# david-mathews-1994/deltarice

Hardware: AMD Instinct MI355X
Metric: encode+decode GB/s (int16 in) (higher is better)
Workload: dtype int16; 1 GPU; 1000000x7000 int16 Gaussian(sigma=10), m=8, 500 chunks of 2000x7000 per GPU, encode then decode, HBM resident; waveforms_per_gpu=1000000, wave_len=7000, rice_m=8, chunks_per_gpu=500, decode_impl=8

## Files before the change

### deltarice_amd/csrc/drx_encode.h

```cpp
#ifndef DRX_ENCODE_H
#define DRX_ENCODE_H
#include <hip/hip_runtime.h>
#include <stdint.h>

#include "drx_device.h"

namespace drx {

constexpr int kTile = 512;

typedef uint16_t u16x2 __attribute__((ext_vector_type(2)));
typedef int16_t i16x2 __attribute__((ext_vector_type(2)));
__device__ __forceinline__ u16x2 as_u16x2(uint32_t x) { return __builtin_bit_cast(u16x2, x); }
__device__ __forceinline__ i16x2 as_i16x2(uint32_t x) { return __builtin_bit_cast(i16x2, x); }
__device__ __forceinline__ uint32_t as_u32(u16x2 x) { return __builtin_bit_cast(uint32_t, x); }
__device__ __forceinline__ u16x2 splat(uint32_t v) { return (u16x2){(uint16_t)v, (uint16_t)v}; }

struct PackedCodes { uint32_t nb[4], c16[4], e[4]; };

template <bool GEN>
__device__ __forceinline__ void packed_codes(const uint32_t x[4], uint32_t xprev, uint32_t xprev2, const u16x2 (&tp)[4],
                                             uint32_t k, PackedCodes &c) {
    const u16x2 kv = splat(k), kp1 = splat(k + 1u), c16k = splat(16u - k);
    const u16x2 mlo = splat((1u << k) - 1u), mdelta = splat(0xffffu - ((1u << k) - 1u));
    u16x2 z[4], qc[4], e[4];
#pragma unroll
    for (int j = 0; j < 4; ++j) {
        const uint32_t xm1 = j ? x[j - 1] : xprev;
        const uint32_t before = __builtin_amdgcn_alignbit(x[j], xm1, 16);
        i16x2 d;
        if (GEN) {
            const uint32_t xm2 = j >= 2 ? x[j - 2] : (j == 1 ? xprev : xprev2);
            const uint32_t before3 = __builtin_amdgcn_alignbit(xm1, xm2, 16);
            d = __builtin_bit_cast(i16x2, (u16x2)(as_u16x2(x[j]) * tp[0] + as_u16x2(before) * tp[1] +
                                                  as_u16x2(xm1) * tp[2] + as_u16x2(before3) * tp[3]));
        } else {
            d = as_i16x2(x[j]) - as_i16x2(before);
        }
        z[j] = __builtin_bit_cast(u16x2, (i16x2)(d << (int16_t)1)) ^
               __builtin_bit_cast(u16x2, (i16x2)(d >> (int16_t)15));
    }
#pragma unroll
    for (int j = 0; j < 4; ++j) qc[j] = __builtin_elementwise_min((u16x2)(z[j] >> kv), splat(8u));
#pragma unroll
    for (int j = 0; j < 4; ++j) e[j] = qc[j] >> (uint16_t)3;
#pragma unroll
    for (int j = 0; j < 4; ++j) c.nb[j] = as_u32(e[j] * c16k + (qc[j] + kp1));
    const uint32_t mword = as_u32(splat(1u << k));
#pragma unroll
    for (int j = 0; j < 4; ++j) {
        const uint32_t mask = as_u32(e[j] * mdelta + mlo);
        c.c16[j] = (mask & as_u32(z[j])) | (~mask & mword);
        c.e[j] = as_u32(e[j]);
    }
}

constexpr uint32_t kEncCapWords = 2048;

__device__ __forceinline__ int load8_dwords(const int16_t *__restrict__ x, uint32_t len, uint32_t t0, int lane,
                                            bool vec_ok, uint32_t w[4]) {
    const uint32_t i0 = t0 + 8u * (uint32_t)lane;
    const int nv = (i0 >= len) ? 0 : (int)((len - i0) < 8u ? (len - i0) : 8u);
    if (vec_ok && nv == 8) {
        const uint4 q = *reinterpret_cast<const uint4 *>(x + i0);
        w[0] = q.x; w[1] = q.y; w[2] = q.z; w[3] = q.w;
    } else {
#pragma unroll
        for (int j = 0; j < 4; ++j) {
            const uint32_t a = (2 * j < nv) ? (uint32_t)(uint16_t)x[i0 + 2 * j] : 0u;
            const uint32_t b = (2 * j + 1 < nv) ? (uint32_t)(uint16_t)x[i0 + 2 * j + 1] : 0u;
            w[j] = a | (b << 16);
        }
    }
    return nv;
}

__device__ __forceinline__ void mask_tail(PackedCodes &c, int nv) {
#pragma unroll
    for (int j = 0; j < 4; ++j) {
        const uint32_t m = (2 * j + 1 < nv) ? 0xffffffffu : ((2 * j < nv) ? 0x0000ffffu : 0u);
        c.nb[j] &= m;
    }
}

__device__ __forceinline__ uint32_t lane_tile_bits(const PackedCodes &c) {
    const u16x2 s = as_u16x2(c.nb[0]) + as_u16x2(c.nb[1]) + as_u16x2(c.nb[2]) + as_u16x2(c.nb[3]);
    const uint32_t v = as_u32(s);
    return (v & 0xffffu) + (v >> 16);
}

template <bool FULL>
__device__ __forceinline__ void emit_tile(const PackedCodes &c, uint32_t pb) {
    typedef uint32_t __attribute__((address_space(3))) lds_u32;
#pragma unroll
    for (int j = 0; j < 8; ++j) {
        const uint32_t n = (j & 1) ? (c.nb[j >> 1] >> 16) : (c.nb[j >> 1] & 0xffffu);
        uint32_t code32 = __builtin_amdgcn_perm(c.e[j >> 1], c.c16[j >> 1], (j & 1) ? 0x07060302u : 0x05040100u);
        if (!FULL) code32 = n ? code32 : 0u;
        const uint32_t pe = pb + n;
        const uint64_t v = (uint64_t)code32 << (((pb & 32u) - pe) & 63u);
        lds_u32 *w = (lds_u32 *)(uintptr_t)((pb >> 3) & ~3u);
        __hip_atomic_fetch_or(w, (uint32_t)(v >> 32), __ATOMIC_RELAXED, __HIP_MEMORY_SCOPE_WORKGROUP);
        if ((uint32_t)v) __hip_atomic_fetch_or(w + 1, (uint32_t)v, __ATOMIC_RELAXED, __HIP_MEMORY_SCOPE_WORKGROUP);
        pb = pe;
    }
}

__device__ __forceinline__ void concat_codes(const PackedCodes &c, uint32_t (&w)[4]) {
    uint32_t w0 = 0, w1 = 0, w2 = 0, w3 = 0;
#pragma unroll
    for (int j = 0; j < 8; ++j) {
        const uint32_t nbj = c.nb[j >> 1];
        const uint32_t n = (j & 1) ? (nbj >> 16) : nbj;
        const uint32_t code32 = __builtin_amdgcn_perm(c.e[j >> 1], c.c16[j >> 1], (j & 1) ? 0x07060302u : 0x05040100u);
        const uint32_t s = 0u - n;
        if (j >= 3) w3 = __builtin_amdgcn_alignbit(w3, w2, s);
        if (j >= 2) w2 = __builtin_amdgcn_alignbit(w2, w1, s);
        if (j >= 1) w1 = __builtin_amdgcn_alignbit(w1, w0, s);
        w0 = (w0 << (n & 31u)) | code32;
    }
    w[0] = w0; w[1] = w1; w[2] = w2; w[3] = w3;
}

__device__ __forceinline__ void place_words(const uint32_t (&wd)[4], uint32_t pe) {
    typedef uint32_t __attribute__((address_space(3))) lds_u32;
    const uint32_t x0 = __builtin_amdgcn_alignbit(wd[0], 0u, pe);
    const uint32_t x1 = __builtin_amdgcn_alignbit(wd[1], wd[0], pe);
    const uint32_t x2 = __builtin_amdgcn_alignbit(wd[2], wd[1], pe);
    const uint32_t x3 = __builtin_amdgcn_alignbit(wd[3], wd[2], pe);
    const uint32_t x4 = __builtin_amdgcn_alignbit(0u, wd[3], pe);
    lds_u32 *w = (lds_u32 *)(uintptr_t)(((pe >> 3) & ~3u) - 16u);
    __hip_atomic_fetch_or(w + 4, x0, __ATOMIC_RELAXED, __HIP_MEMORY_SCOPE_WORKGROUP);
    __hip_atomic_fetch_or(w + 3, x1, __ATOMIC_RELAXED, __HIP_MEMORY_SCOPE_WORKGROUP);
    __hip_atomic_fetch_or(w + 2, x2, __ATOMIC_RELAXED, __HIP_MEMORY_SCOPE_WORKGROUP);
    if (x3 | x4) {
        __hip_atomic_fetch_or(w + 1, x3, __ATOMIC_RELAXED, __HIP_MEMORY_SCOPE_WORKGROUP);
        if (x4) __hip_atomic_fetch_or(w, x4, __ATOMIC_RELAXED, __HIP_MEMORY_SCOPE_WORKGROUP);
    }
}

constexpr uint32_t kBufFront = 4;

__device__ __forceinline__ void zero_row(uint32_t *row, uint32_t words, int lane) {
    for (int i = lane; i < (int)(words / 4u); i += 64) reinterpret_cast<uint4 *>(row)[i] = make_uint4(0, 0, 0, 0);
}

struct TileCodes {
    PackedCodes c;
    uint32_t cw[4], lane_bits, incl, tile_bits;
};

template <bool GEN, bool FULLT>
__device__ __forceinline__ TileCodes code_tile(const uint32_t (&w)[4], int nv, uint32_t &carry, uint32_t &carry2, const u16x2 (&tp)[4],
                                               uint32_t k) {
    TileCodes t;
    const uint32_t xprev = wave_shr1_carry(w[3], carry);
    carry = (uint32_t)__builtin_amdgcn_readlane((int)w[3], 63);
    uint32_t xprev2 = 0;
    if (GEN) {
        xprev2 = wave_shr1_carry(w[2], carry2);
        carry2 = (uint32_t)__builtin_amdgcn_readlane((int)w[2], 63);
    }
    packed_codes<GEN>(w, xprev, xprev2, tp, k, t.c);
    if (!FULLT) mask_tail(t.c, nv);
    t.lane_bits = lane_tile_bits(t.c);
    if (FULLT) concat_codes(t.c, t.cw);
    t.incl = wave_incl_scan_dpp(t.lane_bits);
    t.tile_bits = (uint32_t)__builtin_amdgcn_readlane((int)t.incl, 63);
    return t;
}

template <bool FULLT, typename At>
__device__ __forceinline__ void put_tile(const TileCodes &t, At &&at) {
    if (FULLT && !__any(t.lane_bits > 128u))
        place_words(t.cw, at(t.incl));
    else
        emit_tile<FULLT>(t.c, at(t.incl - t.lane_bits));
}

__device__ __forceinline__ void shr128(uint32_t (&w)[4], uint32_t n) {
    const uint32_t ws = n >> 5;
    const uint32_t y0 = ws == 0u ? w[0] : ws == 1u ? w[1] : ws == 2u ? w[2] : ws == 3u ? w[3] : 0u;
    const uint32_t y1 = ws == 0u ? w[1] : ws == 1u ? w[2] : ws == 2u ? w[3] : 0u;
    const uint32_t y2 = ws == 0u ? w[2] : ws == 1u ? w[3] : 0u;
    const uint32_t y3 = ws == 0u ? w[3] : 0u;
    w[0] = __builtin_amdgcn_alignbit(y1, y0, n);
    w[1] = __builtin_amdgcn_alignbit(y2, y1, n);
    w[2] = __builtin_amdgcn_alignbit(y3, y2, n);
    w[3] = y3 >> (n & 31u);
}

template <bool GEN>
__device__ __forceinline__ TileCodes code_tail_tile(const uint32_t (&w)[4], int nv, bool ragged, uint32_t &carry, uint32_t &carry2,
                                                    const u16x2 (&tp)[4], uint32_t k, bool &wide) {
    TileCodes t;
    const uint32_t xprev = wave_shr1_carry(w[3], carry);
    carry = (uint32_t)__builtin_amdgcn_readlane((int)w[3], 63);
    uint32_t xprev2 = 0;
    if (GEN) {
        xprev2 = wave_shr1_carry(w[2], carry2);
        carry2 = (uint32_t)__builtin_amdgcn_readlane((int)w[2], 63);
    }
    packed_codes<GEN>(w, xprev, xprev2, tp, k, t.c);
    const uint32_t all_bits = lane_tile_bits(t.c);
    concat_codes(t.c, t.cw);
    if (ragged) {
        PackedCodes cm = t.c;
        mask_tail(cm, nv);
        t.lane_bits = lane_tile_bits(cm);
        shr128(t.cw, all_bits - t.lane_bits);
    } else {
        t.lane_bits = nv ? all_bits : 0u;
#pragma unroll
        for (int j = 0; j < 4; ++j) t.cw[j] = nv ? t.cw[j] : 0u;
    }
    wide = __any((nv ? all_bits : 0u) > 128u);
    t.incl = wave_incl_scan_dpp(t.lane_bits);
    t.tile_bits = (uint32_t)__builtin_amdgcn_readlane((int)t.incl, 63);
    return t;
}

template <typename At>
__device__ __forceinline__ void put_tail_tile(const TileCodes &t, int nv, bool wide, At &&at) {
    if (!wide) {
        place_words(t.cw, at(t.incl));
    } else {
        PackedCodes c = t.c;
        mask_tail(c, nv);
        emit_tile<false>(c, at(t.incl - t.lane_bits));
    }
}

template <typename B, typename F>
__device__ __forceinline__ void for_full_tiles(const int16_t *__restrict__ x, uint32_t n_full, int lane, B &&between, F &&full) {
    constexpr int kDepth = 3;
    const uint4 *xv = reinterpret_cast<const uint4 *>(x) + lane;
    uint4 q[kDepth];
    uint32_t t = 0;
#pragma unroll
    for (int u = 0; u < kDepth; ++u) {
        q[u] = make_uint4(0, 0, 0, 0);
        if ((uint32_t)u < n_full) q[u] = xv[64 * (size_t)u];
    }
#pragma unroll 1
    for (; t + 2u * kDepth <= n_full; t += kDepth) {
        between();
#pragma unroll
        for (int u = 0; u < kDepth; ++u) {
            const uint32_t w[4] = {q[u].x, q[u].y, q[u].z, q[u].w};
            full(w);
            q[u] = xv[64 * (size_t)(t + u + kDepth)];
        }
    }
#pragma unroll 1
    for (; t < n_full; t += kDepth) {
        between();
#pragma unroll
        for (int u = 0; u < kDepth; ++u) {
            if (t + (uint32_t)u < n_full) {
                const uint32_t w[4] = {q[u].x, q[u].y, q[u].z, q[u].w};
                full(w);
                if (t + (uint32_t)u + kDepth < n_full) q[u] = xv[64 * (size_t)(t + u + kDepth)];
            }
        }
    }
}

template <typename B, typename F, typename T>
__device__ __forceinline__ void for_tiles(const int16_t *__restrict__ x, uint32_t len, uint32_t n_full, bool tail, int lane,
                                          B &&between, F &&full, T &&tailf) {
    constexpr int kDepth = 3;
    const uint32_t last = tail ? n_full : n_full - 1u;
    const uint32_t imax = len - 8u;
    auto load = [&](uint32_t tile) -> uint4 {
        tile = tile < last ? tile : last;
        uint32_t i = tile * (uint32_t)kTile + 8u * (uint32_t)lane;
        i = i < imax ? i : imax;
        return *reinterpret_cast<const uint4 *>(x + i);
    };
    uint4 q[kDepth];
#pragma unroll
    for (int u = 0; u < kDepth; ++u) {
        q[u] = load((uint32_t)u);
        __builtin_amdgcn_sched_barrier(0);
    }
    uint32_t t = 0;
#pragma unroll 1
    for (; t + kDepth <= n_full; t += kDepth) {
        between(true);
#pragma unroll
        for (int u = 0; u < kDepth; ++u) {
            const uint32_t w[4] = {q[u].x, q[u].y, q[u].z, q[u].w};
            full(w);
            q[u] = load(t + (uint32_t)u + kDepth);
        }
    }
    const uint32_t left = n_full - t;
    static_assert(kDepth == 3, "the straight code below");
    if (left) {
        between(false);
        const uint32_t w0[4] = {q[0].x, q[0].y, q[0].z, q[0].w};
        full(w0);
        if (left > 1u) {
            const uint32_t w1[4] = {q[1].x, q[1].y, q[1].z, q[1].w};
            full(w1);
        }
    }
    if (tail) {
        auto sel = [left](uint32_t a, uint32_t b, uint32_t c) -> uint32_t { return left == 0u ? a : (left == 1u ? b : c); };
        const uint32_t w[4] = {sel(q[0].x, q[1].x, q[2].x), sel(q[0].y, q[1].y, q[2].y), sel(q[0].z, q[1].z, q[2].z),
                               sel(q[0].w, q[1].w, q[2].w)};
        tailf(w);
    } else {
        __builtin_amdgcn_s_waitcnt(0x0f70);
    }
}

template <bool GEN, bool WINDOW>
__device__ __forceinline__ uint64_t recode_tiles(const int16_t *__restrict__ x, uint32_t len, uint32_t carry, uint32_t carry2,
                                                 const u16x2 (&tp)[4], uint32_t k, int lane, uint32_t *row, uint32_t row_words,
                                                 uint32_t *__restrict__ outp, uint32_t P0, uint32_t skip, uint32_t limit, uint64_t cap) {
    zero_row(row, row_words, lane);
    wave_sync();
    uint32_t *buf = row + kBufFront;
    const uint32_t buf_bits = lds_addr(buf) * 8u;
    auto mine = [&](uint64_t idx) -> bool { return !WINDOW || (idx >= skip && idx < limit && idx < cap); };
    uint64_t P = P0;
    uint32_t wn[4];
    int nvn = load8_dwords(x, len, 0u, lane, true, wn);
    for (uint32_t t0 = 0; t0 < len; t0 += kTile) {
        const uint32_t w[4] = {wn[0], wn[1], wn[2], wn[3]};
        const int nv = nvn;
        if (t0 + kTile < len) nvn = load8_dwords(x, len, t0 + kTile, lane, true, wn);
        const TileCodes t = code_tile<GEN, false>(w, nv, carry, carry2, tp, k);
        const uint64_t wfirst = P >> 5;
        const uint32_t at0 = buf_bits + (uint32_t)(P & 31u);
        put_tile<false>(t, [&](uint32_t bit) -> uint32_t { return at0 + bit; });
        P += t.tile_bits;
        wave_sync();
        const uint32_t nfull = (uint32_t)((P >> 5) - wfirst);
        for (uint32_t i = lane; i < nfull; i += 64) {
            if (mine(wfirst + i)) outp[wfirst + i] = buf[i];
            buf[i] = 0;
        }
        wave_sync();
        if (nfull && lane == 0) { const uint32_t cwd = buf[nfull]; buf[nfull] = 0; buf[0] = cwd; }
        wave_sync();
    }
    if (lane == 0) {
        if ((P & 31u) && mine(P >> 5)) outp[P >> 5] = buf[0];
        buf[0] = 0;
    }
    wave_sync();
    return P;
}

template <bool GEN>
__device__ __forceinline__ uint64_t recode_waveform(const int16_t *__restrict__ x, uint32_t len, const u16x2 (&tp)[4], uint32_t k, int lane,
                                                    uint32_t *row, uint32_t row_words, uint32_t *__restrict__ outp) {
    return recode_tiles<GEN, false>(x, len, 0u, 0u, tp, k, lane, row, row_words, outp, 0u, 0u, 0u, 0ull);
}

template <bool GEN>
__device__ __forceinline__ void history_before(const int16_t *__restrict__ x, uint32_t &carry, uint32_t &carry2) {
    carry = (uint32_t)(uint16_t)x[-1] << 16;
    if (GEN) {
        carry |= (uint32_t)(uint16_t)x[-2];
        carry2 = (uint32_t)(uint16_t)x[-4] | ((uint32_t)(uint16_t)x[-3] << 16);
    }
}

template <bool GEN>
__device__ __forceinline__ void recode_range(const int16_t *__restrict__ xw, uint32_t wf_len, uint32_t s_begin, uint32_t s_end, uint64_t Bp,
                                             uint32_t bits_mine, const u16x2 (&tp)[4], uint32_t k, int lane, uint32_t *row,
                                             uint32_t row_words, uint32_t *__restrict__ payload, uint64_t cap_words) {
    const uint32_t P0 = (uint32_t)(Bp & 31u);
    const uint64_t wbase = Bp >> 5;
    const uint32_t more = wf_len - s_end < 32u ? wf_len - s_end : 32u;
    uint32_t carry = 0, carry2 = 0;
    if (s_begin) history_before<GEN>(xw + s_begin, carry, carry2);
    recode_tiles<GEN, true>(xw + s_begin, s_end - s_begin + more, carry, carry2, tp, k, lane, row, row_words, payload + wbase, P0,
                            P0 ? 1u : 0u, (P0 + bits_mine + 31u) >> 5, cap_words > wbase ? cap_words - wbase : 0ull);
}

}
#endif
```

### deltarice_amd/csrc/drx_encode_stream.hip

```cpp
#include <hip/hip_runtime.h>
#include <stdint.h>

#include <type_traits>

#include "drx_internal.h"
#include "drx_device.h"
#include "drx_encode.h"

namespace drx {

constexpr int kEsWaves = 4;
constexpr uint32_t kEsFront = kBufFront;
constexpr uint32_t kEsBack = 12;
constexpr uint64_t kEsFlag = 1ull << 63;
constexpr uint32_t kEsCtrlWords = 32;
constexpr uint32_t kEsRing = kEsRingWords;
constexpr int kEsPollSleep = 4;

__device__ __forceinline__ uint64_t es_load(const uint64_t *p) {
    return __hip_atomic_load(p, __ATOMIC_RELAXED, __HIP_MEMORY_SCOPE_AGENT);
}
__device__ __forceinline__ void es_store(uint64_t *p, uint64_t v) {
    __hip_atomic_store(p, v, __ATOMIC_RELAXED, __HIP_MEMORY_SCOPE_AGENT);
}

constexpr uint32_t kScPer = 8;

__device__ __forceinline__ void es_scanner(uint64_t total, const uint64_t *__restrict__ size, uint64_t *__restrict__ place,
                                           DevStatus *st) {
    const int lane = lane_id();
    if (threadIdx.x >= 64) return;
    __builtin_amdgcn_s_setprio(3);
    uint64_t pos = 0, base = 0;
    uint32_t idle = 0;
    auto sample = [&](uint64_t (&v)[kScPer], uint64_t at) {
#pragma unroll
        for (int j = 0; j < (int)kScPer; ++j) {
            const uint64_t e = at + 64u * j + (uint32_t)lane;
            v[j] = e < total ? es_load(size + e) : kEsFlag;
        }
    };
    while (pos < total) {
        uint64_t v[kScPer];
        const uint64_t bs = pos;
        sample(v, pos);
        uint64_t run = 0;
        bool open = true, big = false;
#pragma unroll
        for (int j = 0; j < (int)kScPer; ++j) {
            const uint64_t e = bs + 64u * j + (uint32_t)lane;
            const uint64_t m = __ballot(e < pos || (v[j] >> 63) != 0);
            const uint32_t l = (m == ~0ull) ? 64u : (uint32_t)__builtin_ctzll(~m);
            run += open ? l : 0u;
            open = open && l == 64u;
            big = big || __any((v[j] & ~kEsFlag) >= (1ull << 24));
        }
        uint64_t end = bs + run;
        end = end < total ? end : total;
        if (end <= pos) {
            if (++idle > (1u << 22)) {
                if (lane == 0) atomicOr(&st->err, kErrInternal);
                return;
            }
            __builtin_amdgcn_s_sleep(1);
            continue;
        }
        idle = 0;
        uint64_t running = 0;
#pragma unroll
        for (int j = 0; j < (int)kScPer; ++j) {
            if (bs + 64u * j < end) {
                const uint64_t e = bs + 64u * j + (uint32_t)lane;
                const bool in = e >= pos && e < end;
                const uint64_t val = in ? (v[j] & ~kEsFlag) : 0ull;
                uint64_t inc;
                if (!big) {
                    inc = wave_incl_scan_dpp((uint32_t)val);
                } else {
                    inc = val;
#pragma unroll
                    for (int d = 1; d < 64; d <<= 1) {
                        const uint64_t t = __shfl_up(inc, d);
                        if (lane >= d) inc += t;
                    }
                }
                if (in) es_store(place + e, kEsFlag | (base + running + inc - val));
                running += big ? __shfl(inc, 63) : (uint64_t)(uint32_t)__builtin_amdgcn_readlane((int)(uint32_t)inc, 63);
            }
        }
        base += running;
        pos = end;
    }
}

template <int WV>
struct EsShared {
    uint32_t role, arrive, ticket[4];
    uint64_t mine[2][WV];
    uint32_t place_t[2];
};

template <int WV>
__device__ __forceinline__ uint32_t es_rendezvous(EsShared<WV> &shm, uint32_t cyc, int lane, int wv, uint32_t *__restrict__ ctrl,
                                                  uint64_t *__restrict__ size, uint32_t Tprev, uint64_t &off) {
    typedef uint32_t __attribute__((address_space(3))) lds_u32;
    uint32_t arr = 0;
    if (lane == 0) arr = __hip_atomic_fetch_add((lds_u32 *)&shm.arrive, 1u, __ATOMIC_RELAXED, __HIP_MEMORY_SCOPE_WORKGROUP);
    arr = (uint32_t)__builtin_amdgcn_readfirstlane((int)arr);
    if (arr == (uint32_t)WV * cyc) {
        if (lane == 0) shm.ticket[cyc & 3u] = atomicAdd(ctrl + 32, 1u);
    }
    __syncthreads();
    const uint32_t T = rfl(shm.ticket[cyc & 3u]);
    if (cyc) {
        uint64_t sum = 0, before = 0;
#pragma unroll
        for (int i = 0; i < WV; ++i) {
            const uint64_t m = rfl64(shm.mine[(cyc - 1u) & 1u][i]);
            sum += m;
            before += i < wv ? m : 0ull;
        }
        off = before;
        if (wv == 0 && lane == 0) es_store(size + Tprev, kEsFlag | sum);
    }
    return T;
}

template <uint32_t RING>
__device__ __forceinline__ uint32_t es_gap(bool pend, uint32_t startA, uint32_t start, uint32_t behind) {
    if (!pend) return RING - 8u;
    const uint32_t d = startA >= start ? startA - start : startA + RING - start;
    return d > behind ? d - behind : 0u;
}

template <typename InLds, typename Wait, typename Copy>
__device__ __forceinline__ bool es_release(bool must, uint64_t P, InLds &&place_in_lds, Wait &&wait_place, Copy &&copy_out) {
    decltype(wait_place()) pl;
    const bool seen = place_in_lds(pl);
    if (!(seen || must)) return false;
    if (!seen) __builtin_amdgcn_s_setprio(0);
    else if (P < (uint64_t)(4u * kTile * 7u)) __builtin_amdgcn_s_setprio(2);
    else __builtin_amdgcn_s_setprio(1);
    copy_out(seen ? pl : wait_place());
    return true;
}

template <uint32_t RING, typename Put>
__device__ __forceinline__ void ring_put_with(const TileCodes &t, uint32_t *row, uint32_t s0, int lane, Put &&put) {
    constexpr uint32_t kRingBits = RING * 32u;
    uint32_t *ring = row + kEsFront;
    const uint32_t ring_bits0 = lds_addr(ring) * 8u;
    put([&](uint32_t bit) -> uint32_t {
        const uint32_t b = s0 + bit;
        return ring_bits0 + (b >= kRingBits ? b - kRingBits : b);
    });
    if (s0 < kRingBits && s0 + t.tile_bits >= kRingBits) {
        wave_sync();
        if (lane < (int)kEsFront) {
            const uint32_t v = row[lane];
            if (v) { ring[RING - kEsFront + lane] |= v; row[lane] = 0; }
        } else if (lane < (int)(kEsFront + kEsBack)) {
            const uint32_t i = (uint32_t)lane - kEsFront, v = ring[RING + i];
            if (v) { ring[i] |= v; ring[RING + i] = 0; }
        }
        wave_sync();
    }
}
template <bool FULLT, uint32_t RING>
__device__ __forceinline__ void ring_put(const TileCodes &t, uint32_t *row, uint32_t s0, int lane) {
    ring_put_with<RING>(t, row, s0, lane, [&](auto &&at) { put_tile<FULLT>(t, at); });
}

static unsigned es_grid(const Geom &G, uint64_t tickets) {
    const unsigned full = 256u * (16u / kEsWaves);
    return (G.dbg & DRX_DBG_STREAM_THREE_WGS) ? 3u : (unsigned)(tickets + 1 < full ? tickets + 1 : full);
}

template <bool GEN, int WV, uint32_t RING>
__global__ __launch_bounds__(64 * WV, 4) void k_encode_stream(Geom G, const int16_t *__restrict__ in, uint32_t *__restrict__ out,
                                                              uint64_t out_cap, uint64_t *__restrict__ chunk_word_off,
                                                              uint32_t *__restrict__ wave_words, uint64_t *__restrict__ size,
                                                              uint64_t *__restrict__ place, uint32_t *__restrict__ ctrl,
                                                              DevStatus *st) {
    __shared__ __attribute__((aligned(16))) uint32_t ring_all[WV][kEsFront + RING + kEsBack];
    __shared__ EsShared<WV> shm;
    __shared__ uint64_t s_place_v[2];
    typedef uint32_t __attribute__((address_space(3))) lds_u32;
    typedef uint64_t __attribute__((address_space(3))) lds_u64;
    static_assert((kEsFront + RING + kEsBack) % 4 == 0 && RING % 4 == 0, "16-byte LDS accesses");
    constexpr uint32_t kRowWords = kEsFront + RING + kEsBack;
    const int lane = lane_id(), wv = wave_id();
    uint32_t *row = ring_all[wv];
    uint32_t *ring = row + kEsFront;

    if (threadIdx.x == 0) {
        shm.role = atomicAdd(ctrl, 1u);
        shm.arrive = 0;
        shm.place_t[0] = shm.place_t[1] = 0;
    }
    zero_row(row, kRowWords, lane);
    __syncthreads();
    const uint64_t n_tickets = (G.total_waves + WV - 1) / WV;
    if (rfl(shm.role) == 0) {
        es_scanner(n_tickets, size, place, st);
        return;
    }

    const uint32_t k = G.k;
    const u16x2 tp[4] = {splat(GEN ? G.enc_t[0] : 1u), splat(GEN ? G.enc_t[1] : 0xffffu), splat(GEN ? G.enc_t[2] : 0u),
                         splat(GEN ? G.enc_t[3] : 0u)};

    bool pend = false, fitsA = true;
    uint64_t gA = 0, offA = 0;
    uint32_t TA = 0, startA = 0, nA = 0;
    WaveRef rA = {};

    auto place_header = [&](const WaveRef &r, uint64_t g, uint32_t n, uint64_t ex, uint64_t &pos) -> bool {
        const uint64_t mine = 1ull + n + (r.idx == 0 ? 1ull : 0ull);
        pos = ex + (r.idx == 0 ? 1ull : 0ull);
        if (lane == 0) {
            if (r.idx == 0) chunk_word_off[r.chunk] = ex;
            if (g + 1 == G.total_waves) {
                chunk_word_off[G.n_chunks] = ex + mine;
                st->total_words = ex + mine;
                if (G.host_words) *G.host_words = ex + mine;
                if (ex + mine > out_cap) atomicOr(&st->err, kErrCapacity);
            }
        }
        const bool room = pos + 1u + n <= out_cap;
        if (room && lane == 0) {
            out[pos] = n;
            if (r.idx == 0) out[pos - 1] = r.n_samples;
        }
        return room;
    };
    auto copy_out = [&](uint64_t ex) {
        uint64_t pos;
        const bool room = place_header(rA, gA, nA, ex + offA, pos);
        uint32_t *__restrict__ outp = out + pos + 1;
        typedef uint32_t u32x4s __attribute__((ext_vector_type(4)));
        typedef u32x4s __attribute__((address_space(1), aligned(4))) g_u32x4_a4;
        const uint32_t n4 = nA & ~3u;
        for (uint32_t i = 4u * (uint32_t)lane; i < n4; i += 256u) {
            uint32_t w = startA + i;
            w = w >= RING ? w - RING : w;
            const uint4 v = *reinterpret_cast<const uint4 *>(ring + w);
            if (room) *(g_u32x4_a4 *)(outp + i) = (u32x4s){v.x, v.y, v.z, v.w};
            *reinterpret_cast<uint4 *>(ring + w) = make_uint4(0, 0, 0, 0);
        }
        if ((uint32_t)lane < nA - n4) {
            uint32_t w = startA + n4 + (uint32_t)lane;
            w = w >= RING ? w - RING : w;
            if (room) outp[n4 + (uint32_t)lane] = ring[w];
            ring[w] = 0;
        }
        wave_sync();
        pend = false;
    };
    auto place_in_lds = [&](uint64_t &ex) -> bool {
        const uint32_t t = __hip_atomic_load((lds_u32 *)&shm.place_t[TA & 1u], __ATOMIC_RELAXED, __HIP_MEMORY_SCOPE_WORKGROUP);
        if (rfl(t) != TA + 1u) return false;
        ex = rfl64(__hip_atomic_load((lds_u64 *)&s_place_v[TA & 1u], __ATOMIC_RELAXED, __HIP_MEMORY_SCOPE_WORKGROUP));
        return true;
    };
    auto place_to_lds = [&](uint64_t ex) {
        if (lane == 0) {
            __hip_atomic_store((lds_u64 *)&s_place_v[TA & 1u], ex, __ATOMIC_RELAXED, __HIP_MEMORY_SCOPE_WORKGROUP);
            __hip_atomic_store((lds_u32 *)&shm.place_t[TA & 1u], TA + 1u, __ATOMIC_RELAXED, __HIP_MEMORY_SCOPE_WORKGROUP);
        }
    };
    auto wait_place = [&]() -> uint64_t {
        uint32_t spins = 0;
        for (;;) {
            uint64_t ex;
            bool have = place_in_lds(ex);
            if (!have) {
                uint64_t v = 0;
                if (lane == 0) v = es_load(place + TA);
                const uint32_t hi = (uint32_t)__builtin_amdgcn_readfirstlane((int)(uint32_t)(v >> 32));
                if (hi >> 31) {
                    ex = ((uint64_t)(hi & 0x7fffffffu) << 32) | (uint32_t)__builtin_amdgcn_readfirstlane((int)(uint32_t)v);
                    place_to_lds(ex);
                    have = true;
                }
            }
            if (have) return ex;
            __builtin_amdgcn_s_sleep(kEsPollSleep);
            if (++spins > (1u << 22)) {
                if (lane == 0) atomicOr(&st->err, kErrInternal);
                return out_cap;
            }
        }
    };

    auto stream_out = [&](uint64_t ex) {
        uint64_t pos;
        const bool room = place_header(rA, gA, nA, ex + offA, pos);
        recode_waveform<GEN>(in + rA.sample_off, room ? rA.len : 0u, tp, k, lane, row, kRowWords, out + pos + 1);
        pend = false;
    };

    uint32_t start = 0;
    uint32_t Tprev = 0;
    for (uint32_t cyc = 0;; ++cyc) {
        const uint32_t T = es_rendezvous(shm, cyc, lane, wv, ctrl, size, Tprev, offA);
        if (pend && !fitsA) stream_out(wait_place());
        if ((uint64_t)T * WV >= G.total_waves) break;
        Tprev = T;
        const uint64_t g = (uint64_t)T * WV + (uint32_t)wv;
        if (g >= G.total_waves) {
            if (lane == 0) shm.mine[cyc & 1u][wv] = 0;
            if (pend) copy_out(wait_place());
            continue;
        }

        const WaveRef r = locate_uniform(G, g);
        const int16_t *x = in + r.sample_off;
        const uint32_t wlen = r.len;
        const uint32_t n_full = wlen / kTile, rem = wlen - n_full * (uint32_t)kTile;
        const bool tail = rem != 0u, ragged = (rem & 7u) != 0u;
        const bool tail_lane = 8u * (uint32_t)lane + 8u <= rem;

        auto gap = [&]() -> uint32_t { return es_gap<RING>(pend, startA, start, 8u); };
        if (pend && gap() < 512u) copy_out(wait_place());
        uint32_t limit = gap();

        uint64_t P = 0;
        bool fits = true;
        uint32_t carry = 0;
        uint32_t carry2 = 0;
        auto process_tile = [&](const uint32_t (&w)[4], int nv, auto full_tag) {
            constexpr bool FULLT = decltype(full_tag)::value;
            bool wide = false;
            TileCodes t;
            if constexpr (FULLT) t = code_tile<GEN, true>(w, nv, carry, carry2, tp, k);
            else t = code_tail_tile<GEN>(w, nv, ragged, carry, carry2, tp, k, wide);
            const uint32_t need = ((uint32_t)P + t.tile_bits + 31u) >> 5;
            bool ok = fits && need < limit;
            if (pend && es_release(fits && !ok, P, place_in_lds, wait_place, copy_out)) {
                limit = gap();
                ok = fits && need < limit;
            }
            if (ok) {
                if constexpr (FULLT) ring_put<true, RING>(t, row, start * 32u + (uint32_t)P, lane);
                else ring_put_with<RING>(t, row, start * 32u + (uint32_t)P, lane, [&](auto &&at) { put_tail_tile(t, nv, wide, at); });
            } else {
                fits = false;
            }
            P += t.tile_bits;
        };
        uint64_t pollv = 0;
        bool polling = false;
        auto between = [&](bool again) {
            if (!pend) return;
            if (polling) {
                const uint32_t hi = (uint32_t)__builtin_amdgcn_readfirstlane((int)(uint32_t)(pollv >> 32));
                polling = false;
                if (hi >> 31) {
                    place_to_lds(((uint64_t)(hi & 0x7fffffffu) << 32) | (uint32_t)__builtin_amdgcn_readfirstlane((int)(uint32_t)pollv));
                    return;
                }
            }
            if (!again) return;
            if (lane == 0) pollv = es_load(place + TA);
            polling = true;
        };

        auto full_tile = [&](const uint32_t (&w)[4]) { process_tile(w, 8, std::true_type{}); };
        auto tail_tile = [&](const uint32_t (&wq)[4]) {
            const uint32_t i0 = 8u * (uint32_t)lane;
            const int nv = tail_lane ? 8 : (i0 < rem ? (int)(rem - i0) : 0);
            uint32_t w[4];
#pragma unroll
            for (int j = 0; j < 4; ++j) w[j] = tail_lane ? wq[j] : 0u;
            if (ragged && nv > 0 && nv < 8) {
                const int16_t *xl = x + (size_t)n_full * kTile + i0;
#pragma unroll
                for (int j = 0; j < 4; ++j) {
                    const uint32_t a = (2 * j < nv) ? (uint32_t)(uint16_t)xl[2 * j] : 0u;
                    const uint32_t b = (2 * j + 1 < nv) ? (uint32_t)(uint16_t)xl[2 * j + 1] : 0u;
                    w[j] = a | (b << 16);
                }
            }
            process_tile(w, nv, std::false_type{});
        };
        if (wlen >= 8u) {
            for_tiles(x, wlen, n_full, tail, lane, between, full_tile, tail_tile);
        } else {
            const uint32_t none[4] = {0u, 0u, 0u, 0u};
            tail_tile(none);
        }
        const uint32_t n = (uint32_t)((P + 31u) >> 5);
        wave_sync();
        if (lane == 0) {
            wave_words[g] = n;
            shm.mine[cyc & 1u][wv] = 1ull + n + (r.idx == 0 ? 1ull : 0ull);
        }
        if (pend) copy_out(wait_place());
        pend = true;
        fitsA = fits;
        gA = g;
        rA = r;
        TA = T;
        startA = start;
        nA = n;
        if (fits) {
            start += (n + 3u) & ~3u;
            start = start >= RING ? start - RING : start;
        }
    }
    if (pend) copy_out(wait_place());
}

struct EsPlace2 { uint64_t whdr, bits; };

__device__ __forceinline__ void es_scanner_segs(uint64_t total, uint32_t tpw, uint32_t waves_per_chunk, const uint64_t *__restrict__ size,
                                                uint64_t *__restrict__ place, DevStatus *st) {
    const int lane = lane_id();
    if (threadIdx.x >= 64) return;
    __builtin_amdgcn_s_setprio(3);
    uint64_t pos = 0;
    uint64_t whdr = 1;
    uint64_t bits_in = 0;
    uint32_t idle = 0;
    const double rcp_tpw = 1.0 / (double)tpw;
    while (pos < total) {
        uint64_t v[kScPer];
        const uint64_t bs = pos;
#pragma unroll
        for (int j = 0; j < (int)kScPer; ++j) {
            const uint64_t e = bs + 64u * j + (uint32_t)lane;
            v[j] = e < total ? es_load(size + e) : 0ull;
        }
        uint64_t run = 0;
        bool open = true;
#pragma unroll
        for (int j = 0; j < (int)kScPer; ++j) {
            const uint64_t m = __ballot((v[j] >> 63) != 0);
            const uint32_t l = (m == ~0ull) ? 64u : (uint32_t)__builtin_ctzll(~m);
            run += open ? l : 0u;
            open = open && l == 64u;
        }
        const uint64_t end = bs + run;
        if (end <= pos) {
            if (++idle > (1u << 22)) {
                if (lane == 0) atomicOr(&st->err, kErrInternal);
                return;
            }
            __builtin_amdgcn_s_sleep(1);
            continue;
        }
        idle = 0;
#pragma unroll
        for (int j = 0; j < (int)kScPer; ++j) {
            if (bs + 64u * j < end) {
                const uint64_t e = bs + 64u * j + (uint32_t)lane;
                const bool in = e < end;
                const uint32_t val = in ? (uint32_t)(v[j] & 0xffffffffull) : 0u;
                const uint32_t e32 = (uint32_t)e;
                uint32_t g = (uint32_t)((double)e32 * rcp_tpw);
                uint32_t jj = e32 - g * tpw;
                if ((int32_t)jj < 0) { g -= 1u; jj += tpw; }
                if (jj >= tpw) { g += 1u; jj -= tpw; }
                const bool closing = in && jj + 1u == tpw;
                const uint32_t inc = wave_incl_scan_dpp(val), ex = inc - val;
                const int f = lane - (int)jj;
                const uint32_t exf = (uint32_t)__shfl((int)ex, f < 0 ? 0 : f);
                const uint64_t before = f < 0 ? bits_in + ex : (uint64_t)(ex - exf);
                const uint64_t nw = closing ? (before + val + 31ull) >> 5 : 0ull;
                const uint64_t contrib = closing ? 1ull + nw + (((g + 1u) % waves_per_chunk == 0u) ? 1ull : 0ull) : 0ull;
                uint64_t cinc;
                if (!__any(contrib >= (1ull << 24))) {
                    cinc = wave_incl_scan_dpp((uint32_t)contrib);
                } else {
                    cinc = contrib;
#pragma unroll
                    for (int d = 1; d < 64; d <<= 1) {
                        const uint64_t t = __shfl_up(cinc, d);
                        if (lane >= d) cinc += t;
                    }
                }
                const uint64_t my_whdr = whdr + cinc - contrib;
                if (in) {
                    es_store(place + 2u * e, kEsFlag | my_whdr);
                    es_store(place + 2u * e + 1u, kEsFlag | before);
                }
                const uint64_t left = end - (bs + 64u * j);
                const int li = __builtin_amdgcn_readfirstlane(left >= 64u ? 63 : (int)left - 1);
                const uint64_t wn = my_whdr + contrib, bn = closing ? 0ull : before + val;
                whdr = ((uint64_t)(uint32_t)__builtin_amdgcn_readlane((int)(uint32_t)(wn >> 32), li) << 32) | (uint32_t)__builtin_amdgcn_readlane((int)(uint32_t)wn, li);
                bits_in = ((uint64_t)(uint32_t)__builtin_amdgcn_readlane((int)(uint32_t)(bn >> 32), li) << 32) | (uint32_t)__builtin_amdgcn_readlane((int)(uint32_t)bn, li);
            }
        }
        pos = end;
    }
}

template <bool GEN, int WV, uint32_t RING>
__global__ __launch_bounds__(64 * WV, 4) void k_encode_stream_segs(Geom G, uint32_t seg_len, uint32_t tpw, const int16_t *__restrict__ in,
                                                                   uint32_t *__restrict__ out, uint64_t out_cap,
                                                                   uint64_t *__restrict__ chunk_word_off, uint32_t *__restrict__ wave_words,
                                                                   uint64_t *__restrict__ size, uint64_t *__restrict__ place,
                                                                   uint32_t *__restrict__ ctrl, DevStatus *st) {
    __shared__ __attribute__((aligned(16))) uint32_t ring_all[WV][kEsFront + RING + kEsBack];
    __shared__ EsShared<WV> shm;
    __shared__ uint64_t s_place_v[2][2];
    __shared__ uint32_t s_first[2][WV];
    typedef uint32_t __attribute__((address_space(3))) lds_u32;
    typedef uint64_t __attribute__((address_space(3))) lds_u64;
    static_assert((kEsFront + RING + kEsBack) % 4 == 0 && RING % 4 == 0, "16-byte LDS accesses");
    static_assert(WV == (int)kEsSegWaves, "es_seg_shape() counts tickets of kEsSegWaves segments");
    constexpr uint32_t kRowWords = kEsFront + RING + kEsBack;
    const int lane = lane_id(), wv = wave_id();
    uint32_t *row = ring_all[wv];
    uint32_t *ring = row + kEsFront;

    if (threadIdx.x == 0) {
        shm.role = atomicAdd(ctrl, 1u);
        shm.arrive = 0;
        shm.place_t[0] = shm.place_t[1] = 0;
    }
    zero_row(row, kRowWords, lane);
    __syncthreads();
    const uint64_t n_tickets = G.total_waves * tpw;
    if (rfl(shm.role) == 0) {
        es_scanner_segs(n_tickets, tpw, G.u_n_waves, size, place, st);
        return;
    }
    const uint32_t k = G.k;
    const u16x2 tp[4] = {splat(GEN ? G.enc_t[0] : 1u), splat(GEN ? G.enc_t[1] : 0xffffu), splat(GEN ? G.enc_t[2] : 0u),
                         splat(GEN ? G.enc_t[3] : 0u)};

    bool pend = false, fitsA = true, lastA = false, sibA = false;
    uint64_t gA = 0, offA = 0;
    uint32_t TA = 0, startA = 0, nA = 0, bitsA = 0, sbeginA = 0, sendA = 0, parA = 0;
    WaveRef rA = {};

    auto headers = [&](const WaveRef &r, const EsPlace2 &pl, uint64_t B) {
        if (lane != 0) return;
        if (sbeginA == 0u && r.idx == 0u) {
            chunk_word_off[r.chunk] = pl.whdr - 1u;
            if (pl.whdr - 1u < out_cap) out[pl.whdr - 1u] = r.n_samples;
        }
        if (lastA) {
            const uint64_t n = (B + bitsA + 31ull) >> 5;
            wave_words[gA] = (uint32_t)n;
            if (pl.whdr < out_cap) out[pl.whdr] = (uint32_t)n;
            if (gA + 1u == G.total_waves) {
                const uint64_t tot = pl.whdr + 1ull + n;
                chunk_word_off[G.n_chunks] = tot;
                st->total_words = tot;
                if (G.host_words) *G.host_words = tot;
                if (tot > out_cap) atomicOr(&st->err, kErrCapacity);
            }
        }
    };
    auto copy_out = [&](const EsPlace2 &pl) {
        const uint64_t B = pl.bits + offA;
        headers(rA, pl, B);
        const uint64_t w0 = pl.whdr + 1ull + (B >> 5);
        const uint32_t s = (uint32_t)B & 31u;
        const uint32_t i_lo = s ? 1u : 0u, i_hi = (s + bitsA + 31u) >> 5;
        const uint32_t nA4 = (nA + 3u) & ~3u, top = nA4 > i_hi ? nA4 : ((i_hi + 3u) & ~3u);
        if (sibA) {
            if (lane == 0) {
                const uint32_t F = s_first[parA][wv + 1], sh = bitsA & 31u;
                uint32_t wi = startA + (bitsA >> 5);
                wi = wi >= RING ? wi - RING : wi;
                ring[wi] |= F >> sh;
                if (sh) {
                    wi = wi + 1u >= RING ? wi + 1u - RING : wi + 1u;
                    ring[wi] |= F << (32u - sh);
                }
            }
            wave_sync();
        }
        uint32_t *__restrict__ outp = out + w0;
        const uint64_t room = out_cap > w0 ? out_cap - w0 : 0ull;
        typedef uint32_t u32x4s __attribute__((ext_vector_type(4)));
        typedef u32x4s __attribute__((address_space(1), aligned(4))) g_u32x4_a4;
        uint32_t carryw = 0;
        for (uint32_t i0 = 0; i0 < top; i0 += 256u) {
            const uint32_t i = i0 + 4u * (uint32_t)lane;
            uint4 v = make_uint4(0, 0, 0, 0);
            uint32_t w = startA + i;
            w = w >= RING ? w - RING : w;
            const bool inr = i < nA4;
            if (inr) v = *reinterpret_cast<const uint4 *>(ring + w);
            uint32_t pw = (uint32_t)__builtin_amdgcn_update_dpp(0, (int)v.w, 0x138, 0xf, 0xf, false);
            if (lane == 0) pw = carryw;
            carryw = (uint32_t)__builtin_amdgcn_readlane((int)v.w, 63);
            const uint32_t o0 = __builtin_amdgcn_alignbit(pw, v.x, s), o1 = __builtin_amdgcn_alignbit(v.x, v.y, s);
            const uint32_t o2 = __builtin_amdgcn_alignbit(v.y, v.z, s), o3 = __builtin_amdgcn_alignbit(v.z, v.w, s);
            if (i >= i_lo && i + 4u <= i_hi && (uint64_t)i + 4u <= room) {
                *(g_u32x4_a4 *)(outp + i) = (u32x4s){o0, o1, o2, o3};
            } else {
                if (i >= i_lo && i < i_hi && (uint64_t)i < room) outp[i] = o0;
                if (i + 1u >= i_lo && i + 1u < i_hi && (uint64_t)i + 1u < room) outp[i + 1u] = o1;
                if (i + 2u >= i_lo && i + 2u < i_hi && (uint64_t)i + 2u < room) outp[i + 2u] = o2;
                if (i + 3u >= i_lo && i + 3u < i_hi && (uint64_t)i + 3u < room) outp[i + 3u] = o3;
            }
            if (inr) *reinterpret_cast<uint4 *>(ring + w) = make_uint4(0, 0, 0, 0);
        }
        wave_sync();
        pend = false;
    };
    auto place_in_lds = [&](EsPlace2 &pl) -> bool {
        const uint32_t t = __hip_atomic_load((lds_u32 *)&shm.place_t[TA & 1u], __ATOMIC_RELAXED, __HIP_MEMORY_SCOPE_WORKGROUP);
        if (rfl(t) != TA + 1u) return false;
        pl.whdr = rfl64(__hip_atomic_load((lds_u64 *)&s_place_v[TA & 1u][0], __ATOMIC_RELAXED, __HIP_MEMORY_SCOPE_WORKGROUP));
        pl.bits = rfl64(__hip_atomic_load((lds_u64 *)&s_place_v[TA & 1u][1], __ATOMIC_RELAXED, __HIP_MEMORY_SCOPE_WORKGROUP));
        return true;
    };
    auto place_to_lds = [&](const EsPlace2 &pl) {
        if (lane == 0) {
            __hip_atomic_store((lds_u64 *)&s_place_v[TA & 1u][0], pl.whdr, __ATOMIC_RELAXED, __HIP_MEMORY_SCOPE_WORKGROUP);
            __hip_atomic_store((lds_u64 *)&s_place_v[TA & 1u][1], pl.bits, __ATOMIC_RELAXED, __HIP_MEMORY_SCOPE_WORKGROUP);
            __hip_atomic_store((lds_u32 *)&shm.place_t[TA & 1u], TA + 1u, __ATOMIC_RELAXED, __HIP_MEMORY_SCOPE_WORKGROUP);
        }
    };
    auto place_of = [&](uint64_t pv, EsPlace2 &pl) -> bool {
        const uint32_t lo = (uint32_t)pv, hi = (uint32_t)(pv >> 32);
        const uint32_t h0 = (uint32_t)__builtin_amdgcn_readlane((int)hi, 0), h1 = (uint32_t)__builtin_amdgcn_readlane((int)hi, 1);
        if (!((h0 & h1) >> 31)) return false;
        pl.whdr = ((uint64_t)(h0 & 0x7fffffffu) << 32) | (uint32_t)__builtin_amdgcn_readlane((int)lo, 0);
        pl.bits = ((uint64_t)(h1 & 0x7fffffffu) << 32) | (uint32_t)__builtin_amdgcn_readlane((int)lo, 1);
        return true;
    };
    auto wait_place = [&]() -> EsPlace2 {
        uint32_t spins = 0;
        for (;;) {
            EsPlace2 pl;
            if (place_in_lds(pl)) return pl;
            uint64_t pv = 0;
            if (lane < 2) pv = es_load(place + 2ull * TA + (uint32_t)lane);
            if (place_of(pv, pl)) {
                place_to_lds(pl);
                return pl;
            }
            __builtin_amdgcn_s_sleep(kEsPollSleep);
            if (++spins > (1u << 22)) {
                if (lane == 0) atomicOr(&st->err, kErrInternal);
                pl.whdr = out_cap;
                pl.bits = 0;
                return pl;
            }
        }
    };

    auto stream_out = [&](const EsPlace2 &pl) {
        const uint64_t B = pl.bits + offA;
        headers(rA, pl, B);
        recode_range<GEN>(in + rA.sample_off, rA.len, sbeginA, sendA, B, bitsA, tp, k, lane, row, kRowWords, out + pl.whdr + 1ull,
                          out_cap > pl.whdr + 1ull ? out_cap - pl.whdr - 1ull : 0ull);
        pend = false;
    };

    uint32_t start = 0;
    uint32_t Tprev = 0;
    for (uint32_t cyc = 0;; ++cyc) {
        const uint32_t T = es_rendezvous(shm, cyc, lane, wv, ctrl, size, Tprev, offA);
        if (pend && !fitsA) stream_out(wait_place());
        if ((uint64_t)T >= n_tickets) break;
        Tprev = T;
        const uint32_t gw = T / tpw, tj = T - gw * tpw;
        const uint64_t g = gw;
        const WaveRef r = locate_uniform(G, g);
        const uint32_t wlen = r.len;
        const uint32_t sgi = tj * (uint32_t)WV + (uint32_t)wv;
        const uint64_t sb64 = (uint64_t)sgi * seg_len;
        if (sb64 >= wlen) {
            if (lane == 0) shm.mine[cyc & 1u][wv] = 0;
            if (pend) copy_out(wait_place());
            continue;
        }
        const uint32_t s_begin = (uint32_t)sb64;
        const uint32_t s_end = wlen - s_begin > seg_len ? s_begin + seg_len : wlen;
        const bool sib = wv + 1 < WV && seg_len >= 32u && wlen - s_end >= 32u;
        const uint32_t more = sib ? 0u : (wlen - s_end < 32u ? wlen - s_end : 32u);
        const uint32_t slen = s_end - s_begin;
        const uint32_t clen = slen + more;
        const int16_t *x = in + r.sample_off + s_begin;

        auto gap = [&]() -> uint32_t { return es_gap<RING>(pend, startA, start, 12u); };
        if (pend && gap() < 512u) copy_out(wait_place());
        uint32_t limit = gap();

        uint64_t P = 0;
        uint32_t seg_bits = 0;
        bool first = true;
        bool fits = true;
        uint32_t carry = 0, carry2 = 0;
        if (s_begin) history_before<GEN>(x, carry, carry2);
        auto process_tile = [&](const uint32_t (&w)[4], int nv, int mark, auto full_tag) {
            constexpr bool FULLT = decltype(full_tag)::value;
            const TileCodes t = code_tile<GEN, FULLT>(w, nv, carry, carry2, tp, k);
            if (!FULLT && mark >= 0) seg_bits = (uint32_t)P + (mark ? (uint32_t)__builtin_amdgcn_readlane((int)t.incl, mark - 1) : 0u);
            const uint32_t need = ((uint32_t)P + t.tile_bits + 31u) >> 5;
            bool ok = fits && need < limit;
            if (pend && es_release(fits && !ok, P, place_in_lds, wait_place, copy_out)) {
                limit = gap();
                ok = fits && need < limit;
            }
            if (ok)
                ring_put<FULLT, RING>(t, row, start * 32u + (uint32_t)P, lane);
            else
                fits = false;
            P += t.tile_bits;
            if (first) {
                first = false;
                wave_sync();
                if (lane == 0) s_first[cyc & 1u][wv] = ring[start];
            }
        };
        const uint32_t n_fast = more ? slen / kTile : clen / kTile;
        uint64_t pollv = 0;
        bool polling = false;
        auto between = [&]() {
            if (!pend) return;
            if (polling) {
                polling = false;
                EsPlace2 pl;
                if (place_of(pollv, pl)) {
                    place_to_lds(pl);
                    return;
                }
            }
            pollv = 0;
            if (lane < 2) pollv = es_load(place + 2ull * TA + (uint32_t)lane);
            polling = true;
        };
        for_full_tiles(x, n_fast, lane, between, [&](const uint32_t (&w)[4]) { process_tile(w, 8, -1, std::true_type{}); });
        for (uint32_t t0 = n_fast * kTile; t0 < clen; t0 += kTile) {
            uint32_t w[4];
            const int nv = load8_dwords(x, clen, t0, lane, true, w);
            const int mark = (more && slen >= t0 && slen < t0 + (uint32_t)kTile) ? (int)((slen - t0) >> 3) : -1;
            process_tile(w, nv, mark, std::false_type{});
        }
        if (!more) seg_bits = (uint32_t)P;
        const uint32_t n = (uint32_t)((P + (sib ? 63u : 31u)) >> 5);
        wave_sync();
        if (lane == 0) shm.mine[cyc & 1u][wv] = seg_bits;
        if (pend) copy_out(wait_place());
        pend = true;
        fitsA = fits;
        gA = g;
        rA = r;
        TA = T;
        startA = start;
        nA = fits ? n : 0u;
        bitsA = seg_bits;
        sbeginA = s_begin;
        sendA = s_end;
        lastA = s_end == wlen;
        sibA = sib;
        parA = cyc & 1u;
        if (fits) {
            start += (n + 3u) & ~3u;
            start = start >= RING ? start - RING : start;
        }
    }
    if (pend) copy_out(wait_place());
}

hipError_t launch_encode_stream(const EncodeCall &c, uint64_t *d_scan) {
    const Geom &G = *c.G;
    const EncOut &o = c.out;
    const hipStream_t s = c.s;
    if (G.total_waves == 0) return hipSuccess;
    const uint64_t W = G.total_waves;
    const uint64_t tickets = (W + kEsWaves - 1) / kEsWaves;
    mark(c.ev, 0, s);
    hipError_t e = hipMemsetAsync(d_scan, 0, (2 * tickets + kEsCtrlWords) * sizeof(uint64_t), s);
    if (e != hipSuccess) return e;
    mark(c.ev, 1, s);
    mark(c.ev, 2, s);
    uint64_t *size = d_scan, *place = d_scan + tickets;
    uint32_t *ctrl = reinterpret_cast<uint32_t *>(d_scan + 2 * tickets);
    const unsigned grid = es_grid(G, tickets);
    if (G.n_taps)
        k_encode_stream<true, kEsWaves, kEsRing><<<grid, 64 * kEsWaves, 0, s>>>(G, c.d_in, o.d_out, o.out_cap, o.d_chunk_word_off, o.d_wave_words,
                                                                              size, place, ctrl, c.d_status);
    else
        k_encode_stream<false, kEsWaves, kEsRing><<<grid, 64 * kEsWaves, 0, s>>>(G, c.d_in, o.d_out, o.out_cap, o.d_chunk_word_off, o.d_wave_words,
                                                                               size, place, ctrl, c.d_status);
    mark(c.ev, 3, s);
    return hipGetLastError();
}

hipError_t launch_encode_stream_segs(const EncodeCall &c, uint32_t seg_target, uint64_t *d_scan) {
    const Geom &G = *c.G;
    const EncOut &o = c.out;
    const hipStream_t s = c.s;
    if (G.total_waves == 0) return hipSuccess;
    const EsSegShape sh = es_seg_shape(G.u_wave_len, seg_target);
    const uint64_t tickets = G.total_waves * sh.tpw;
    mark(c.ev, 0, s);
    hipError_t e = hipMemsetAsync(d_scan, 0, (3 * tickets + kEsCtrlWords) * sizeof(uint64_t), s);
    if (e != hipSuccess) return e;
    mark(c.ev, 1, s);
    mark(c.ev, 2, s);
    uint64_t *size = d_scan, *place = d_scan + tickets;
    uint32_t *ctrl = reinterpret_cast<uint32_t *>(d_scan + 3 * tickets);
    const unsigned grid = es_grid(G, tickets);
    if (G.n_taps)
        k_encode_stream_segs<true, kEsWaves, kEsRing><<<grid, 64 * kEsWaves, 0, s>>>(G, sh.seg_len, sh.tpw, c.d_in, o.d_out, o.out_cap, o.d_chunk_word_off,
                                                                                   o.d_wave_words, size, place, ctrl, c.d_status);
    else
        k_encode_stream_segs<false, kEsWaves, kEsRing><<<grid, 64 * kEsWaves, 0, s>>>(G, sh.seg_len, sh.tpw, c.d_in, o.d_out, o.out_cap, o.d_chunk_word_off,
                                                                                    o.d_wave_words, size, place, ctrl, c.d_status);
    mark(c.ev, 3, s);
    return hipGetLastError();
}

}
```

Before: 1575 GB/s.

## Deepen tile prefetch to four, force VGPR params, unconditional second LDS OR

```diff
diff --git a/deltarice_amd/csrc/drx_encode.h b/deltarice_amd/csrc/drx_encode.h
--- a/deltarice_amd/csrc/drx_encode.h
+++ b/deltarice_amd/csrc/drx_encode.h
@@ -89,7 +89,7 @@
     return (v & 0xffffu) + (v >> 16);
 }
 
-template <bool FULL>
+template <bool FULL, bool BOTH = false>
 __device__ __forceinline__ void emit_tile(const PackedCodes &c, uint32_t pb) {
     typedef uint32_t __attribute__((address_space(3))) lds_u32;
 #pragma unroll
@@ -101,7 +101,7 @@
         const uint64_t v = (uint64_t)code32 << (((pb & 32u) - pe) & 63u);
         lds_u32 *w = (lds_u32 *)(uintptr_t)((pb >> 3) & ~3u);
         __hip_atomic_fetch_or(w, (uint32_t)(v >> 32), __ATOMIC_RELAXED, __HIP_MEMORY_SCOPE_WORKGROUP);
-        if ((uint32_t)v) __hip_atomic_fetch_or(w + 1, (uint32_t)v, __ATOMIC_RELAXED, __HIP_MEMORY_SCOPE_WORKGROUP);
+        if (BOTH || (uint32_t)v) __hip_atomic_fetch_or(w + 1, (uint32_t)v, __ATOMIC_RELAXED, __HIP_MEMORY_SCOPE_WORKGROUP);
         pb = pe;
     }
 }
@@ -170,12 +170,12 @@
     return t;
 }
 
-template <bool FULLT, typename At>
+template <bool FULLT, bool BOTH = false, typename At>
 __device__ __forceinline__ void put_tile(const TileCodes &t, At &&at) {
     if (FULLT && !__any(t.lane_bits > 128u))
         place_words(t.cw, at(t.incl));
     else
-        emit_tile<FULLT>(t.c, at(t.incl - t.lane_bits));
+        emit_tile<FULLT, BOTH>(t.c, at(t.incl - t.lane_bits));
 }
 
 __device__ __forceinline__ void shr128(uint32_t (&w)[4], uint32_t n) {
@@ -220,14 +220,14 @@
     return t;
 }
 
-template <typename At>
+template <bool BOTH = false, typename At>
 __device__ __forceinline__ void put_tail_tile(const TileCodes &t, int nv, bool wide, At &&at) {
     if (!wide) {
         place_words(t.cw, at(t.incl));
     } else {
         PackedCodes c = t.c;
         mask_tail(c, nv);
-        emit_tile<false>(c, at(t.incl - t.lane_bits));
+        emit_tile<false, BOTH>(c, at(t.incl - t.lane_bits));
     }
 }
 
@@ -269,7 +269,7 @@
 template <typename B, typename F, typename T>
 __device__ __forceinline__ void for_tiles(const int16_t *__restrict__ x, uint32_t len, uint32_t n_full, bool tail, int lane,
                                           B &&between, F &&full, T &&tailf) {
-    constexpr int kDepth = 3;
+    constexpr int kDepth = 4;
     const uint32_t last = tail ? n_full : n_full - 1u;
     const uint32_t imax = len - 8u;
     auto load = [&](uint32_t tile) -> uint4 {
@@ -296,20 +296,25 @@
         }
     }
     const uint32_t left = n_full - t;
-    static_assert(kDepth == 3, "the straight code below");
     if (left) {
         between(false);
-        const uint32_t w0[4] = {q[0].x, q[0].y, q[0].z, q[0].w};
-        full(w0);
-        if (left > 1u) {
-            const uint32_t w1[4] = {q[1].x, q[1].y, q[1].z, q[1].w};
-            full(w1);
+#pragma unroll
+        for (int u = 0; u < kDepth - 1; ++u) {
+            if ((uint32_t)u < left) {
+                const uint32_t w[4] = {q[u].x, q[u].y, q[u].z, q[u].w};
+                full(w);
+            }
         }
     }
     if (tail) {
-        auto sel = [left](uint32_t a, uint32_t b, uint32_t c) -> uint32_t { return left == 0u ? a : (left == 1u ? b : c); };
-        const uint32_t w[4] = {sel(q[0].x, q[1].x, q[2].x), sel(q[0].y, q[1].y, q[2].y), sel(q[0].z, q[1].z, q[2].z),
-                               sel(q[0].w, q[1].w, q[2].w)};
+        uint32_t w[4] = {q[kDepth - 1].x, q[kDepth - 1].y, q[kDepth - 1].z, q[kDepth - 1].w};
+#pragma unroll
+        for (int u = kDepth - 2; u >= 0; --u) {
+            w[0] = left == (uint32_t)u ? q[u].x : w[0];
+            w[1] = left == (uint32_t)u ? q[u].y : w[1];
+            w[2] = left == (uint32_t)u ? q[u].z : w[2];
+            w[3] = left == (uint32_t)u ? q[u].w : w[3];
+        }
         tailf(w);
     } else {
         __builtin_amdgcn_s_waitcnt(0x0f70);
diff --git a/deltarice_amd/csrc/drx_encode_stream.hip b/deltarice_amd/csrc/drx_encode_stream.hip
--- a/deltarice_amd/csrc/drx_encode_stream.hip
+++ b/deltarice_amd/csrc/drx_encode_stream.hip
@@ -206,9 +206,10 @@
         return;
     }
 
-    const uint32_t k = G.k;
-    const u16x2 tp[4] = {splat(GEN ? G.enc_t[0] : 1u), splat(GEN ? G.enc_t[1] : 0xffffu), splat(GEN ? G.enc_t[2] : 0u),
-                         splat(GEN ? G.enc_t[3] : 0u)};
+    uint32_t k = G.k, et[4] = {GEN ? G.enc_t[0] : 1u, GEN ? G.enc_t[1] : 0xffffu, GEN ? G.enc_t[2] : 0u, GEN ? G.enc_t[3] : 0u};
+    asm volatile("" : "+v"(k));
+    if (GEN) asm volatile("" : "+v"(et[0]), "+v"(et[1]), "+v"(et[2]), "+v"(et[3]));
+    const u16x2 tp[4] = {splat(et[0]), splat(et[1]), splat(et[2]), splat(et[3])};
 
     bool pend = false, fitsA = true;
     uint64_t gA = 0, offA = 0;
@@ -342,8 +343,8 @@
                 ok = fits && need < limit;
             }
             if (ok) {
-                if constexpr (FULLT) ring_put<true, RING>(t, row, start * 32u + (uint32_t)P, lane);
-                else ring_put_with<RING>(t, row, start * 32u + (uint32_t)P, lane, [&](auto &&at) { put_tail_tile(t, nv, wide, at); });
+                if constexpr (FULLT) ring_put_with<RING>(t, row, start * 32u + (uint32_t)P, lane, [&](auto &&at) { put_tile<true, true>(t, at); });
+                else ring_put_with<RING>(t, row, start * 32u + (uint32_t)P, lane, [&](auto &&at) { put_tail_tile<true>(t, nv, wide, at); });
             } else {
                 fits = false;
             }
```

New measurement: 1589 GB/s (median of 6 runs). No clear change (+0.9%).
